# lrm2017/Fastest_Image_Pattern_Matching

Measured on AMD Instinct MI355X. Metric: template matches/sec + ms/search, 4024×3036 src ±180°; HBM GB/s vs roofline, higher is better.
Workload: dtype u8

## Files before the change

### fastest_image_pattern_matching_amd/csrc/fpm_engine.hip

```cpp
#include <hip/hip_runtime.h>

#include <algorithm>
#include <array>
#include <cfloat>
#include <chrono>
#include <cmath>
#include <cstdio>
#include <cstdlib>
#include <cstring>
#include <new>
#include <random>
#include <string>
#include <vector>

#include "../../include/fpm.h"
#include "fpm_host.h"
#include "fpm_kernels.h"
#include "fpm_model.h"

using namespace fpm;

namespace {

inline int round_up(int v, int a) { return (v + a - 1) / a * a; }
// ... 64 lines not shown
    std::vector<size_t> node_off;
    F2 center;
    std::vector<size_t> canvas_off, map_off, blk_off;
    std::vector<int> canvas_pitch, map_w, map_h, nblk;
    std::vector<int32_t> order;
    size_t canvas_bytes = 0, map_floats = 0, blk_count = 0;
    int max_canvas = 0, max_map = 0, max_nblk = 0, max_cells = 0, max_nitems = 0;
    NmsMaxima nmax;
    int off_skey = 0, nzero = 0;
    bool top_mma = false;
    TopMmaArgs tma{};
    int tcand_cap = 0;
    DevBuf d_tmu, d_tcandv;
    DevBuf d_ncand;
    DevBuf d_canvas, d_map, d_bmax, d_bloc, d_jobs, d_nodes, d_top, d_topn, d_peaks, d_counts, d_state,
        d_live, d_livecnt, d_rec, d_rowsum, d_wsum, d_wsq, d_tab, d_roi, d_tdesc, d_state2, d_rec2;
    int tabw = 0, tabh = 0, roi_pitch = 0, tdesc_stride = 1;
    size_t roi_stride = 0;
    int slot_cap = 0;
    size_t off_warp = 0, off_ncc = 0, off_nms = 0, off_order = 0;
    PinBuf h_out;
    size_t h_counts = 0, h_peaks = 0, h_live = 0, h_live0 = 0, h_state = 0, h_rec = 0, h_total = 0;
    char* h_dev = nullptr;
    void release() {
        for (DevBuf* b : {&d_tmu, &d_tcandv, &d_ncand, &d_canvas, &d_map, &d_bmax, &d_bloc, &d_jobs, &d_nodes, &d_top, &d_topn, &d_peaks,
                          &d_counts, &d_state, &d_live, &d_livecnt, &d_rec, &d_rowsum, &d_wsum, &d_wsq, &d_tab, &d_roi, &d_tdesc, &d_state2, &d_rec2})
            b->release();
        h_out.release();
        valid = false;
    }
};

struct RawPose {
    float x, y;
    double angle;
};

struct KProf {
    std::vector<std::pair<hipEvent_t, hipEvent_t>> ev;
    size_t used = 0;
    double ms = 0;
// ... 11 lines not shown
    bool learned = false;
    int border = 0;
    std::vector<TmplLevel> tmpl;
    DevBuf d_tmpl, d_tmpl8, d_tsum;
    uint64_t tmpl_gen = 0;
    int S = 0, sw = 0, sh = 0, src_L = -1;
    int shard = 0, shards = 1;
    std::vector<SrcLevel> src;
    DevBuf d_src;
    PinBuf h_imgtab;
    DevBuf d_imgtab;
    hipEvent_t in_ev = nullptr;
    Plan plan;
    uint64_t plan_gen = ~0ull;
    DevBuf d_op_a, d_op_b, d_op_job;
    DevBuf d_rf_tab, d_rf_tdesc, d_rf_roi, d_rf_rowsum, d_rf_wsum, d_rf_wsq;
    DevBuf d_ov;
    PinBuf h_ov_in, h_ov_out;
    std::vector<int64_t> stats;
    int64_t alg_bytes[3] = {0, 0, 0};
    bool prof = false;
    KProf kp[kProfSlots];
    hipGraphExec_t graph = nullptr;
    uint64_t graph_plan = ~0ull;
    const void* graph_src = nullptr;
    uint64_t plan_builds = 0;
    hipEvent_t t_ev[2] = {nullptr, nullptr};
    double last_device_ms = 0, last_host_ms = 0, last_call_ms = 0;
    std::chrono::steady_clock::time_point t_call0;
    bool pending = false;
    bool staged = false;
// ... 131 lines not shown
    n.cn = std::cos(-r); n.sn = std::sin(-r);
    return n;
}

SrcLevel level_layout(int w, int h) {
    SrcLevel s{};
    s.w = w; s.h = h;
    s.pitch = round_up(w + 4, 64);
    s.img_bytes = round_up((size_t)s.pitch * (h + 1), (size_t)256);
    return s;
}
size_t level_slab_slack(int pitch0) { return 16 * (size_t)pitch0 + 256; }

struct RoiScratchDims {
    int tabw = 1, tabh = 1, roi_pitch = 1, tdesc_stride = 1;
    size_t roi_stride = 0, max_rows = 1, max_chunks = 1;
    size_t per_roi() const {
        return sizeof(int32_t) * 2 * (tabw + tabh) + sizeof(int4) * tdesc_stride + roi_stride + max_rows * 49 * 4 +
               max_chunks * 49 * 12;
    }
};
RoiScratchDims roi_scratch_dims(const TmplLevel* lv, int nlv) {
    RoiScratchDims d;
    int max_w = 1;
    for (int l = 0; l < nlv; ++l) {
        d.tdesc_stride = std::max(d.tdesc_stride, roi_tiles_for(lv[l].w, lv[l].h));
        const int rc = roi_pick_rc(lv[l].w, lv[l].h);
        d.max_rows = std::max(d.max_rows, (size_t)lv[l].h);
        d.max_chunks = std::max(d.max_chunks, (size_t)(lv[l].h + rc - 1) / rc);
        max_w = std::max(max_w, lv[l].w);
        d.roi_stride = std::max(d.roi_stride, roi_tiles_bytes(lv[l].w, lv[l].h));
    }
    d.roi_pitch = roi_pitch_for(max_w);
    d.tabw = d.roi_pitch;
    d.tabh = roi_tab_rows((int)d.max_rows);
    return d;
}
hipError_t roi_scratch_ensure(const RoiScratchDims& d, size_t slots, DevBuf& tab, DevBuf& tdesc, DevBuf& roi,
                              DevBuf& rowsum, DevBuf& wsum, DevBuf& wsq) {
    hipError_t e = tab.ensure(slots * 2 * (d.tabw + d.tabh) * sizeof(int32_t));
    if (e == hipSuccess) e = tdesc.ensure(slots * d.tdesc_stride * sizeof(int4));
    if (e == hipSuccess) e = roi.ensure(slots * d.roi_stride);
    if (e == hipSuccess) e = rowsum.ensure(slots * round_up(d.max_rows * 49, (size_t)4) * 4);
    if (e == hipSuccess) e = wsum.ensure(slots * d.max_chunks * 49 * 4);
    if (e == hipSuccess) e = wsq.ensure(slots * d.max_chunks * 49 * 8);
    return e;
}

bool same_search_params(const fpm_params& a, const fpm_params& b) {
    return a.max_pos == b.max_pos && a.min_reduce_area == b.min_reduce_area && a.max_overlap == b.max_overlap &&
           a.score == b.score && a.tolerance_angle == b.tolerance_angle && a.use_simd == b.use_simd &&
           a.tolerance_range == b.tolerance_range && a.semantics == b.semantics &&
           a.top_angle_step == b.top_angle_step && std::equal(a.tolerance, a.tolerance + 4, b.tolerance) &&
           (a.stop_layer != 0) == (b.stop_layer != 0);
}

constexpr double kMaxTopAngles = 100000;
static bool angle_list_ok(const fpm_params& prm, double step, bool mfc) {
    if (!std::isfinite(step) || step <= 0) return false;
    auto span = [&](double lo, double hi) { return (hi - lo) / step + 2; };
// ... 246 lines not shown
        P.tabw = rd.tabw;
        P.tabh = rd.tabh;
        P.roi_stride = rd.roi_stride;
        const size_t per_roi = rd.per_roi();
        size_t free_b = 0, total_b = 0;
        if (hipMemGetInfo(&free_b, &total_b) != hipSuccess) free_b = (size_t)16 << 30;
        size_t budget = std::min((size_t)48 << 30, std::max(std::min((size_t)4 << 30, free_b / 2), free_b / 6));
        if (const char* e = getenv("FPM_SCRATCH_MB")) {
            const long mb = atol(e);
            if (mb > 0) budget = std::min(budget, (size_t)mb << 20);
        }
        const size_t want = (size_t)P.C * P.n3;
        P.slot_cap = (int)std::max<size_t>((size_t)P.n3, std::min(want, budget / per_roi) / P.n3 * P.n3);
        for (;;) {
            const hipError_t e = roi_scratch_ensure(rd, (size_t)P.slot_cap, P.d_tab, P.d_tdesc, P.d_roi, P.d_rowsum,
                                                    P.d_wsum, P.d_wsq);
            if (e == hipSuccess) break;
            (void)hipGetLastError();
            if (e != hipErrorOutOfMemory || P.slot_cap <= P.n3) HIP_TRY(e);
            P.d_tab.release(); P.d_tdesc.release(); P.d_roi.release();
            P.d_rowsum.release(); P.d_wsum.release(); P.d_wsq.release();
            P.slot_cap = std::max(P.n3, P.slot_cap / 2 / P.n3 * P.n3);
        }
    }
    std::vector<WarpJob> wj(J);
    std::vector<NccJob> nj(J);
    std::vector<NmsJob> mj(J);
    const uint8_t* dsrc = ctx->d_src.as<uint8_t>();
    for (int s = 0; s < S; ++s)
        for (int a = 0; a < P.nang; ++a) {
            const int k = s * P.nang + a;
            uint8_t* canvas = P.d_canvas.as<uint8_t>() + P.canvas_bytes * s + P.canvas_off[a];
            float* map = P.d_map.as<float>() + P.map_floats * s + P.map_off[a];
            WarpJob& w = wj[k];
            w.src = dsrc + top.off + top.img_bytes * s;
            w.sw = top.w; w.sh = top.h; w.sp = top.pitch;
// ... 294 lines not shown
    const char* stab_env = getenv("FPM_STEP_TABLES");
    const bool step_tables = (stab_env ? atoi(stab_env) != 0 : true) && (size_t)P.C * P.n3 <= (size_t)P.slot_cap;
    bool tables_done = false;
    for (int l = L - 1; l >= stop; --l) {
        const int d = L - 1 - l;
        const SrcLevel& lv = ctx->src[l];
        const TmplLevel& tl = ctx->tmpl[l];
        const bool in_run = l >= run_end;
        RoiArgs ra{};
        ra.level = dsrc + lv.off; ra.level_stride = lv.img_bytes;
        ra.W = lv.w; ra.H = lv.h; ra.P = lv.pitch;
        ra.tmpl = ctx->d_tmpl.as<uint8_t>() + tl.off; ra.tw = tl.w; ra.th = tl.h; ra.tp = tl.pitch;
        ra.tmpl8 = ctx->d_tmpl8.as<int8_t>() + tl.off8; ra.tp8 = tl.p8; ra.nk = (tl.w + 63) / 64;
        ra.tsum = ctx->d_tsum.as<int32_t>() + tl.tsum_off;
        ra.n3 = P.n3;
        ra.rc = roi_pick_rc(tl.w, tl.h);
        ra.nchunk = (tl.h + ra.rc - 1) / ra.rc;
        ra.fold = ctx->prm.use_simd ? 1 : 0;
        ra.equal1 = tl.equal1 ? 1 : 0;
        ra.per_source = P.nang * P.cap;
        ra.mean = tl.mean; ra.norm = tl.norm; ra.inv_area = tl.inv_area;
        ra.live = live[cur_list];
        ra.live_count = livecnt + list_cnt;
        ra.state = P.d_state.as<CandState>();
        ra.nodes = P.d_nodes.as<AngleNode>() + P.node_off[d];
        ra.tab = P.d_tab.as<int32_t>(); ra.tabw = roi_pitch_for(tl.w); ra.tabh = roi_tab_rows(tl.h);
        ra.tdesc = P.d_tdesc.as<int4>(); ra.tdesc_stride = P.tdesc_stride;
        ra.roi = P.d_roi.as<uint8_t>(); ra.roi_pitch = roi_pitch_for(tl.w); ra.roi_stride = P.roi_stride;
        ra.rowsum = P.d_rowsum.as<uint32_t>();
        ra.wsum = P.d_wsum.as<uint32_t>();
        ra.wsq = P.d_wsq.as<uint64_t>();
        ra.rec = P.d_rec.as<RoiRecord>();
        ra.step = l > stop ? 1 : 0;
        ra.mark_reached0 = l - 1 == stop ? 1 : 0;
        ra.live_out = live[cur_list ^ 1];
        ra.live_out_count = livecnt + d + 1;
        ra.thr = P.layer_score[l];
        if (in_run) {
            ra.rec = rec_buf[run_k & 1];
            if (run_k > 0) {
                ra.state = state_buf[(run_k + 1) & 1];
                ra.state_out = state_buf[run_k & 1];
                ra.prev_rec = rec_buf[(run_k + 1) & 1];
                ra.prev_nodes = P.d_nodes.as<AngleNode>() + P.node_off[d - 1];
                ra.prev_thr = P.layer_score[l + 1];
                ra.prev_W = ctx->src[l + 1].w;
// ... 1517 lines not shown
    }
    *out = ctx;
    return FPM_OK;
}

int fpm_destroy(fpm_ctx* ctx) {
    if (!ctx) return FPM_E_INVALID_ARG;
    (void)hipSetDevice(ctx->device);
    (void)hipStreamSynchronize(ctx->stream);
    if (ctx->graph) (void)hipGraphExecDestroy(ctx->graph);
    for (hipEvent_t e : ctx->t_ev)
        if (e) (void)hipEventDestroy(e);
    ctx->plan.release();
    ctx->d_tmpl.release(); ctx->d_tmpl8.release(); ctx->d_tsum.release(); ctx->d_src.release();
    ctx->d_op_a.release(); ctx->d_op_b.release(); ctx->d_op_job.release();
    for (DevBuf* b : {&ctx->d_rf_tab, &ctx->d_rf_tdesc, &ctx->d_rf_roi, &ctx->d_rf_rowsum, &ctx->d_rf_wsum, &ctx->d_rf_wsq})
        b->release();
    ctx->d_ov.release(); ctx->h_ov_in.release(); ctx->h_ov_out.release();
    ctx->d_imgtab.release(); ctx->h_imgtab.release();
    if (ctx->in_ev) (void)hipEventDestroy(ctx->in_ev);
    ctx->d_patchtab.release(); ctx->h_patchtab.release(); ctx->d_patch.release();
    ctx->d_cmpacc.release(); ctx->h_cmpacc.release();
    ctx->d_tacc.release(); ctx->h_tacc.release();
    ctx->d_model.release(); ctx->d_band.release(); ctx->d_insacc.release(); ctx->h_insacc.release();
    ctx->d_alnacc.release(); ctx->h_alnacc.release();
    for (hipEvent_t e : {ctx->tab_ev, ctx->out_ev})
        if (e) (void)hipEventDestroy(e);
    for (auto& k : ctx->kp)
        for (auto& e : k.ev) { (void)hipEventDestroy(e.first); (void)hipEventDestroy(e.second); }
    (void)hipStreamDestroy(ctx->stream);
    delete ctx;
// ... 1017 lines not shown
    hl[C] = C;
    const size_t o_state = 0, o_live = round_up(sizeof(CandState) * C, (size_t)256),
                 o_nodes = o_live + round_up(sizeof(int32_t) * (C + 1), (size_t)256),
                 o_rec = o_nodes + round_up(sizeof(AngleNode) * total_rois, (size_t)256);
    HIP_TRY(ctx->d_op_b.ensure(o_rec + sizeof(RoiRecord) * (size_t)total_rois));
    HIP_TRY(hipMemcpyAsync(ctx->d_op_b.as<char>(o_state), hs.data(), sizeof(CandState) * C, hipMemcpyHostToDevice, st));
    HIP_TRY(hipMemcpyAsync(ctx->d_op_b.as<char>(o_live), hl.data(), sizeof(int32_t) * (C + 1), hipMemcpyHostToDevice, st));
    HIP_TRY(hipMemcpyAsync(ctx->d_op_b.as<char>(o_nodes), hn.data(), sizeof(AngleNode) * total_rois, hipMemcpyHostToDevice,
                           st));
    HIP_TRY(hipMemsetAsync(ctx->d_op_b.as<char>(o_rec), 0, sizeof(RoiRecord) * (size_t)total_rois, st));
    const int slot_cap = round_rois > 0 ? std::min(round_rois, total_rois) : total_rois;
    const bool small = roi_small_fits(tl.w, tl.h);
    const RoiScratchDims rd = roi_scratch_dims(&tl, 1);
    if (!small)
        HIP_TRY(roi_scratch_ensure(rd, (size_t)slot_cap, ctx->d_rf_tab, ctx->d_rf_tdesc, ctx->d_rf_roi, ctx->d_rf_rowsum,
                                   ctx->d_rf_wsum, ctx->d_rf_wsq));
    RoiArgs ra{};
    ra.level = ctx->d_op_a.as<uint8_t>(); ra.level_stride = lv.img_bytes;
    ra.W = lv.w; ra.H = lv.h; ra.P = lv.pitch;
    ra.tmpl = ctx->d_tmpl.as<uint8_t>() + tl.off; ra.tw = tl.w; ra.th = tl.h; ra.tp = tl.pitch;
    ra.tmpl8 = ctx->d_tmpl8.as<int8_t>() + tl.off8; ra.tp8 = tl.p8; ra.nk = (tl.w + 63) / 64;
    ra.tsum = ctx->d_tsum.as<int32_t>() + tl.tsum_off;
    ra.n3 = n3;
    ra.rc = roi_pick_rc(tl.w, tl.h);
    ra.nchunk = (tl.h + ra.rc - 1) / ra.rc;
    ra.fold = fold ? 1 : 0;
    ra.equal1 = tl.equal1 ? 1 : 0;
    ra.per_source = n;
    ra.mean = tl.mean; ra.norm = tl.norm; ra.inv_area = tl.inv_area;
    ra.live = ctx->d_op_b.as<int32_t>(o_live);
    ra.live_count = ra.live + C;
    ra.state = ctx->d_op_b.as<CandState>(o_state);
    ra.nodes = ctx->d_op_b.as<AngleNode>(o_nodes);
    ra.tab = ctx->d_rf_tab.as<int32_t>(); ra.tabw = roi_pitch_for(tl.w); ra.tabh = roi_tab_rows(tl.h);
    ra.tdesc = ctx->d_rf_tdesc.as<int4>(); ra.tdesc_stride = rd.tdesc_stride;
    ra.roi = ctx->d_rf_roi.as<uint8_t>(); ra.roi_pitch = roi_pitch_for(tl.w); ra.roi_stride = rd.roi_stride;
    ra.rowsum = ctx->d_rf_rowsum.as<uint32_t>();
    ra.wsum = ctx->d_rf_wsum.as<uint32_t>();
    ra.wsq = ctx->d_rf_wsq.as<uint64_t>();
    ra.rec = ctx->d_op_b.as<RoiRecord>(o_rec);
    ra.step = 0;
    const bool want_px = roi_pixels && !small && !tl.equal1;
    const int RW = tl.w + 6, RH = tl.h + 6, txn = (RW + 31) / 32;
    std::vector<uint8_t> tiles;
    for (int base = 0; base < total_rois; base += slot_cap) {
        ra.slot_base = base;
        ra.slot_cap = std::min(slot_cap, total_rois - base);
        if (small) {
            ProfScope ps(ctx, FPM_K_ROI_SMALL, 0);
            launch_roi_small(ra, st);
            continue;
        }
        {
            ProfScope ps(ctx, FPM_K_ROI_TABLES, 0);
// ... 426 lines not shown
```

### fastest_image_pattern_matching_amd/csrc/fpm_kernels.h

```cpp
#pragma once
#include <hip/hip_runtime.h>
#include <stdint.h>

#include "fpm_geom.h"

namespace fpm {

struct WarpJob {
    const uint8_t* src;
    uint8_t* dst;
    int32_t sw, sh, sp;
    int32_t dw, dh, dp;
    int32_t border;
    int32_t pad;
    double M[6];
};

struct NccJob {
    const uint8_t* img;
    const uint8_t* tmpl;
    float* out;
    int32_t iw, ih, ip;
    int32_t tw, th, tp;
    int32_t ow, oh;
// ... 62 lines not shown
    F2 center;
    int32_t refine;
};

struct RoiArgs {
    const uint8_t* level;
    size_t level_stride;
    int32_t W, H, P;
    const uint8_t* tmpl;
    int32_t tw, th, tp;
    const int8_t* tmpl8;
    int32_t tp8;
    int32_t nk;
    const int32_t* tsum;
    int32_t n3;
    int32_t rc;
    int32_t nchunk;
    int32_t fold;
    int32_t equal1;
    int32_t per_source;
    int32_t slot_base;
    int32_t slot_cap;
    double mean, norm, inv_area;
    const int32_t* live;
    const int32_t* live_count;
    CandState* state;
    const AngleNode* nodes;
    int32_t* tab;
    int32_t tabw, tabh;
    int4* tdesc;
    int32_t tdesc_stride;
    uint8_t* roi;
    int32_t roi_pitch;
    size_t roi_stride;
    int32_t nparts;
    uint32_t* rowsum;
    uint32_t* wsum;
    uint64_t* wsq;
    RoiRecord* rec;
    int32_t step;
    int32_t mark_reached0;
    int32_t* live_out;
    int32_t* live_out_count;
    double thr;
    const RoiRecord* prev_rec;
    const AngleNode* prev_nodes;
    double prev_thr;
    int32_t prev_W, prev_H;
    CandState* state_out;
    int32_t* nt_tab;
    const AngleNode* nt_nodes;
    int32_t nt_tabw, nt_tabh, nt_tw, nt_th, nt_W, nt_H;
    uint64_t* stamps;
// ... 199 lines not shown
                       NmsLaunchInfo* info = nullptr);
void launch_roi_tables(const RoiArgs& a, hipStream_t st);
void launch_roi_warp(const RoiArgs& a, hipStream_t st);
void launch_roi_corr(const RoiArgs& a, hipStream_t st);
void launch_roi_eval(const RoiArgs& a, hipStream_t st);
bool roi_small_fits(int tw, int th);
size_t roi_small_lds(int tw, int th);
void launch_roi_small(const RoiArgs& a, hipStream_t st);
void launch_cand_step(const RoiArgs& a, int max_items, hipStream_t st);
void launch_pack(const PackArgs& a, hipStream_t st);

struct OvRect { F2 c[4]; float w, h; };
constexpr int kOverlapMaxCand = 512;
void launch_overlap_pairs(const OvRect* r, const float4* box, int n, double max_overlap, int32_t* lists, int list_cap,
                          int32_t* offcnt, int32_t* meta, hipStream_t st);
int roi_pick_rc(int tw, int th);
int roi_pitch_for(int tw);
int roi_tab_rows(int th);
size_t roi_tiles_bytes(int tw, int th);
int roi_tiles_for(int tw, int th);
size_t roi_corr_lds(int roi_pitch, int tw, int rc);
constexpr int kMmaRows = 16;

}
```

### fastest_image_pattern_matching_amd/csrc/fpm_kernels.hip

```cpp
#include <float.h>
#include <stdio.h>
#include <stdlib.h>
#include <limits.h>

#include <map>
#include <mutex>
#include <type_traits>
#include <utility>

#include "../../include/fpm.h"
#include "fpm_kernels.h"
#include "fpm_model.h"
#include "fpm_rrect.h"

static void ensure_lds_attr(const void* fn, size_t bytes) {
    if (bytes <= 65536) return;
    int dev = 0;
    (void)hipGetDevice(&dev);
    static std::mutex mu;
    static std::map<std::pair<int, const void*>, size_t> done;
    std::lock_guard<std::mutex> lock(mu);
    size_t& cur = done[std::make_pair(dev, fn)];
    if (bytes <= cur) return;
    (void)hipFuncSetAttribute(fn, hipFuncAttributeMaxDynamicSharedMemorySize, (int)bytes);
// ... 2036 lines not shown
    const int mode = !fuse ? 0 : (ci->refine == 0 ? 1 : (ci->refine == 2 ? 3 : 2));
    if (fuse && zero && nzero > 0 && mode != 1) {
        std::fprintf(stderr, "fpm: launch_top_fused contract violated (counter zeroing with candidate-init mode %d)\n",
                     mode);
        std::abort();
    }
    const int grid = top_fused_grid(njobs_n);
    if (dump)
        hipLaunchKernelGGL(k_top_fused<true>, dim3(grid), dim3(kTopThreads), lds, st, wjobs, njobs, a, zero, nzero,
                           fuse ? *ci : cz, mode, order, njobs_n);
    else
        hipLaunchKernelGGL(k_top_fused<false>, dim3(grid), dim3(kTopThreads), lds, st, wjobs, njobs, a, zero, nzero,
                           fuse ? *ci : cz, mode, order, njobs_n);
}

constexpr int ROI_RC = kMmaRows;
constexpr int ROI_T = 32;
constexpr int ROI_FT = 4096;
constexpr int kFtPitch = 68;
constexpr int kTabShift = 6;
constexpr int kTabFrac = kAbBits + kTabShift;
constexpr int kTapShift = kTabFrac - kInterBits;
constexpr uint32_t kRoiFlip = 0x80808080u;

int roi_pick_rc(int , int th) { return th < ROI_RC ? th : ROI_RC; }

__host__ __device__ inline int roi_pitch_calc(int tw) {
    const int need_a = tw + 6 + 16, need_b = 64 * ((tw + 63) / 64) + 22;
    int q = ((need_a > need_b ? need_a : need_b) + 15) / 16;
    if ((q & 1) == 0) ++q;
    return q * 16;
}
int roi_pitch_for(int tw) { return roi_pitch_calc(tw); }
int roi_tab_rows(int th) { return (th + 6 + ROI_T - 1) / ROI_T * ROI_T; }
__host__ __device__ inline int roi_tab_row_pos(int y) { return (y & ~31) | ((y & 7) << 2) | ((y >> 3) & 3); }
size_t roi_tiles_bytes(int tw, int th) {
    return (size_t)((tw + 6 + ROI_T - 1) / ROI_T) * ((th + 6 + ROI_T - 1) / ROI_T) * ROI_T * ROI_T;
}

__host__ __device__ inline int tmpl_lds_pitch(int tp8) {
    int q = tp8 / 16;
    if ((q & 1) == 0) ++q;
    return q * 16;
}

size_t roi_corr_lds(int roi_pitch, int , int ) {
    constexpr int src_rows = 2 * kMmaRows + 6;
    return (size_t)src_rows * roi_pitch +
           sizeof(uint32_t) * (2 * src_rows + 2 * 7 * src_rows + 2 * kMmaRows + 2 * kMmaRows * 49) + 64;
}

__device__ __forceinline__ int roi_tap(const uint8_t* __restrict__ src, int sw, int sh, int sp, int X, int Y) {
    const int sx = sat_s16(X >> kInterBits), sy = sat_s16(Y >> kInterBits);
    const int fx = X & (kInterTab - 1), fy = Y & (kInterTab - 1);
    int v0, v1, v2, v3;
    if ((unsigned)sx < (unsigned)(sw - 1) && (unsigned)sy < (unsigned)(sh - 1)) {
        const uint8_t* p = src + (size_t)sy * sp + sx;
        v0 = p[0]; v1 = p[1]; v2 = p[sp]; v3 = p[sp + 1];
    } else if (sx >= sw || sx + 1 < 0 || sy >= sh || sy + 1 < 0) {
        return 0;
    } else {
// ... 1472 lines not shown
    p1 = __builtin_amdgcn_udot4(a1, 0x01010101u, p1, false);
    p1 = __builtin_amdgcn_udot4(b0, 0x01010101u, p1, false);
    p1 = __builtin_amdgcn_udot4(b1, 0x01010101u, p1, false);
    uint32_t m1 = __builtin_amdgcn_udot4(c0, 0x01010101u, 0u, false);
    m1 = __builtin_amdgcn_udot4(c1, 0x01010101u, m1, false);
    uint32_t p2 = __builtin_amdgcn_udot4(a0, a0, 0u, false);
    p2 = __builtin_amdgcn_udot4(a1, a1, p2, false);
    p2 = __builtin_amdgcn_udot4(b0, b0, p2, false);
    p2 = __builtin_amdgcn_udot4(b1, b1, p2, false);
    uint32_t m2 = __builtin_amdgcn_udot4(c0, c0, 0u, false);
    m2 = __builtin_amdgcn_udot4(c1, c1, m2, false);
    q1 = p1 - m1;
    q2 = p2 - m2;
}

#ifndef FPM_CORR_PRIO
#define FPM_CORR_PRIO 1
#endif
template <int MODE, int WPE, int NK = 0, bool PFR = true, int RS = 1, bool SE = false, bool DMA = false>
__global__ __launch_bounds__(256) __attribute__((amdgpu_waves_per_eu(WPE))) void k_roi_corr(RoiArgs a) {
    static_assert(!DMA || (NK > 0 && !PFR), "LDS-DMA staging replaces the register staging of the register-A form");
    static_assert(NK == 0 || MODE != 3, "the staging ablation belongs to the slot-major form");
    static_assert(RS == 1 || RS == 3 || RS == 4, "the row statistics' forms");
    static_assert(!SE || NK > 0, "the staged epilogue is flushed in the register-A form's staging phase");
    static_assert(RS < 3 || NK > 0, "the matrix-core row sums read the register-A form's staged rows, every byte defined");
    extern __shared__ __attribute__((aligned(16))) uint8_t smem[];
    const int tw = a.tw, th = a.th, RW = tw + 6;
    const int SBp = a.roi_pitch;
    uint8_t* const SB = smem;
    uint32_t* wi = (uint32_t*)(SB + (size_t)kBandSrc * SBp) + 2 * kBandSrc;
    uint32_t* wq = wi + kBandSrc * 7;
    uint32_t* lts = wq + kBandSrc * 7;
    uint32_t* rsb = lts + 2 * kMmaRows;
    const int tid = threadIdx.x, lane = tid & 63, wv = tid >> 6;
    const int nband = (th + kBandRows - 1) / kBandRows;
    const int rois = roi_count(a), items = rois * nband;
    const int q4 = SBp >> 4;
    const int nwr = (RW + 3) >> 2;
    const int g = lane >> 4, n = lane & 15;
    const int mt = wv & 1, nt = mt + (wv >> 1);
    const int txn = (RW + ROI_T - 1) / ROI_T;
    const int npad = max(0, (min(ROI_T * txn, 64 * a.nk) - 4 * nwr) >> 2);
    const XcdSplit xs = xcd_split(items);
    int it_lo = xs.lo + xs.k, it_hi = xs.hi, it_step = xs.nk;
// ... 126 lines not shown
            uint32_t* rw = (uint32_t*)(SB + (size_t)sr * SBp);
            if (npad > 0) {
                if (g3 < npad) rw[nwr + g3] = kRoiFlip;
                if (g3 + 4 < npad) rw[nwr + g3 + 4] = kRoiFlip;
            }
            const int wr = tw >> 2;
            const uint32_t l0 = rw[0], l1 = rw[1], x0 = rw[wr], x1 = rw[wr + 1], x2 = rw[wr + 2];
            uint32_t s1, s2;
            tile_row_sums<RS == 4>((const uint8_t*)rw + 16 * g3, a.nk, n3, s1, s2);
            s2 = (uint32_t)__shfl((int)s2, n3 + 16 * (n3 >> 2), 64);
            const uint32_t e0 = __builtin_amdgcn_alignbyte(x1, x0, (uint32_t)tw) ^ 0x80808080u;
            const uint32_t e1 = __builtin_amdgcn_alignbyte(x2, x1, (uint32_t)tw) ^ 0x80808080u;
            const uint64_t lo = (uint64_t)(l0 ^ 0x80808080u) | ((uint64_t)(l1 ^ 0x80808080u) << 32);
            const uint64_t hi = (uint64_t)e0 | ((uint64_t)e1 << 32);
            const int nf = min(6, 64 * a.nk - tw);
#pragma unroll
            for (int h = 0; h < 2; ++h) {
                const int dx = g3 + 4 * h;
                if (dx < 7 && row < nsrc) {
                    uint32_t q1, q2;
                    window_edges(lo, hi, dx, nf, q1, q2);
                    wi[row * 7 + dx] = s1 - q1;
                    wq[row * 7 + dx] = s2 - q2;
                }
            }
        }
        if (RS == 1 && MODE != 7 && tid < 4 * nsrc) {
            const int r = tid >> 2, qq = tid & 3;
            const int per = (nwr + 3) >> 2, k0 = qq * per, k1 = min(nwr, k0 + per);
            const uint32_t* row = (const uint32_t*)(SB + (size_t)r * SBp);
            uint32_t s1 = 0, s2 = 0;
            int k = k0;
            for (; k + 8 <= k1; k += 8) {
                uint32_t x[8];
#pragma unroll
                for (int u = 0; u < 8; ++u) x[u] = row[k + u] ^ 0x80808080u;
#pragma unroll
                for (int u = 0; u < 8; ++u) {
                    s1 = __builtin_amdgcn_udot4(x[u], 0x01010101u, s1, false);
                    s2 = __builtin_amdgcn_udot4(x[u], x[u], s2, false);
                }
// ... 17 lines not shown
                const int dx = qq + 4 * h;
                if (dx < 7) {
                    const uint32_t ml0 = dx >= 4 ? 0xffffffffu : (1u << (8 * dx)) - 1u;
                    const uint32_t ml1 = dx <= 4 ? 0u : (1u << (8 * (dx - 4))) - 1u;
                    const uint32_t mr0 = dx >= 4 ? 0u : ~((1u << (8 * dx)) - 1u);
                    const uint32_t mr1 = dx <= 4 ? 0xffffu : dx == 5 ? 0xff00u : 0u;
                    const uint32_t a0 = l0 & ml0, a1 = l1 & ml1, b0 = e0 & mr0, b1 = e1 & mr1;
                    uint32_t q1 = __builtin_amdgcn_udot4(a0, 0x01010101u, 0u, false);
                    q1 = __builtin_amdgcn_udot4(a1, 0x01010101u, q1, false);
                    q1 = __builtin_amdgcn_udot4(b0, 0x01010101u, q1, false);
                    q1 = __builtin_amdgcn_udot4(b1, 0x01010101u, q1, false);
                    uint32_t q2 = __builtin_amdgcn_udot4(a0, a0, 0u, false);
                    q2 = __builtin_amdgcn_udot4(a1, a1, q2, false);
                    q2 = __builtin_amdgcn_udot4(b0, b0, q2, false);
                    q2 = __builtin_amdgcn_udot4(b1, b1, q2, false);
                    wi[r * 7 + dx] = s1 - q1;
                    wq[r * 7 + dx] = s2 - q2;
                }
            }
        }
        __syncthreads();
        auto partials = [&]() {
            if (MODE == 6 || tid >= 4 * 49) return;
            const int pr = tid >> 1, half = tid & 1;
            const int h = pr / 49, k = pr - h * 49;
            const int chunk = (T0 >> 4) + h;
            const int tlo = kMmaRows * h, thi = min(tlo + kMmaRows, rb);
            const bool ok = chunk < a.nchunk && tlo < thi;
            const int pdy = k / 7, ddx = k - pdy * 7;
            const int t0 = tlo + 8 * half, n8 = ok ? min(8, thi - t0) : 0;
            uint32_t s1 = 0, x[8], y[8];
#pragma unroll
            for (int u = 0; u < 8; ++u) {
                const int i = (t0 + u + pdy) * 7 + ddx;
                x[u] = u < n8 ? wi[i] : 0u;
                y[u] = u < n8 ? wq[i] : 0u;
            }
            uint64_t s2 = 0;
#pragma unroll
            for (int u = 0; u < 8; ++u) { s1 += x[u]; s2 += y[u]; }
            s1 += (uint32_t)__builtin_amdgcn_mov_dpp((int)s1, 0xB1, 0xF, 0xF, false);
            const uint32_t lo = (uint32_t)s2, hi = (uint32_t)(s2 >> 32);
            s2 += (uint64_t)(uint32_t)__builtin_amdgcn_mov_dpp((int)lo, 0xB1, 0xF, 0xF, false) |
                  ((uint64_t)(uint32_t)__builtin_amdgcn_mov_dpp((int)hi, 0xB1, 0xF, 0xF, false) << 32);
            if (ok && half == 0) {
                uint32_t kk = (uint32_t)k;
                asm volatile("" : "+v"(kk));
                const uint32_t wo = ((uint32_t)slot * (uint32_t)a.nchunk + (uint32_t)chunk) * 49u + kk;
                a.wsum[wo] = s1;
                a.wsq[wo] = s2;
            }
        };
        const bool active = kMmaRows * mt < rb && kMmaRows * nt < nsrc;
        if (FPM_CORR_PRIO == 1) __builtin_amdgcn_s_setprio(1);
        if (MODE != 2 && active) {
            int sr = kMmaRows * nt + n;
            if (sr >= nsrc) sr = 0;
            const uint8_t* bp = SB + (size_t)sr * SBp + 16 * g;
            fpm_v4i acc[7];
            if (FPM_CORR_PRIO == 2) __builtin_amdgcn_s_setprio(1);
            if (NK > 0)
                band_mfma_regs<NA>(Areg, bp, a.nk, acc);
            else
                band_mfma_ga(a.tmpl8 + (size_t)(T0 + kMmaRows * mt + n) * a.tp8 + 16 * g, bp, a.nk, acc);
            if (FPM_CORR_PRIO == 2) __builtin_amdgcn_s_setprio(0);
            uint32_t* rs_out = a.rowsum + (((size_t)th * 49 + 3) & ~(size_t)3) * slot + (size_t)T0 * 49;
// ... 14 lines not shown
                        if (x == 0x9e3779b9u && a.W < 0) rs_out[t] = x;
                        continue;
                    }
                    const uint32_t o = (uint32_t)(t * 49 + dy * 7);
                    if (SE) {
#pragma unroll
                        for (int d = 0; d < 7; ++d) rsb[o + d] = (uint32_t)acc[d][r] + 128u * (wi[s_ * 7 + d] + ts) - kFix;
                        continue;
                    }
#pragma unroll
                    for (int d = 0; d < 7; ++d) rs_out[o + d] = (uint32_t)acc[d][r] + 128u * (wi[s_ * 7 + d] + ts) - kFix;
                }
            }
        }
        if (FPM_CORR_PRIO == 1) __builtin_amdgcn_s_setprio(0);
        partials();
        if (SE) { pv_slot = slot; pv_T0 = T0; pv_rb = rb; }
    }
    if (SE && pv_slot >= 0) {
        __syncthreads();
        flush();
    }
}

__device__ __forceinline__ CandState cand_step_state(CandState s, int n3, const AngleNode* nodes, double thr, int W,
                                                     int H, int mark_reached0, const float* score, const int* mx,
                                                     const int* my, const AngleNode* next_nodes = nullptr,
                                                     int jj = 0, AngleNode* next_nd = nullptr, int nnext = 1) {
    int imax = 0;
    double big = -1;
    for (int k = 0; k < n3; ++k)
// ... 479 lines not shown
                         RoiRecord* keep) {
    constexpr int kEvalRows = ROWS, kEvalDma = EvalBlk<ROWS>::dma, kEvalBuf = EvalBlk<ROWS>::buf;
    const int th = a.th;
    if (a.equal1) {
        if (lane == 0) {
            RoiRecord r;
            r.score = 1.f; r.mx = 0; r.my = 0; r.on_border = 1;
            for (int k = 0; k < 9; ++k) r.vec[k] = 0.f;
            *out = r;
            *keep = r;
        }
        return;
    }
    const size_t total4 = ((size_t)th * 49 + 3) >> 2;
    const uint4* rs = (const uint4*)(a.rowsum + (size_t)slot * total4 * 4);
    uint64_t s1 = 0, s2 = 0;
    if (lane < 49) {
        const uint32_t* ws = a.wsum + (size_t)slot * a.nchunk * 49 + lane;
        const uint64_t* wq = a.wsq + (size_t)slot * a.nchunk * 49 + lane;
        int c = 0;
        for (; c + 8 <= a.nchunk; c += 8) {
            uint32_t x[8];
            uint64_t y[8];
#pragma unroll
            for (int u = 0; u < 8; ++u) { x[u] = ws[(size_t)(c + u) * 49]; y[u] = wq[(size_t)(c + u) * 49]; }
#pragma unroll
            for (int u = 0; u < 8; ++u) { s1 += x[u]; s2 += y[u]; }
        }
        for (; c < a.nchunk; ++c) { s1 += ws[(size_t)c * 49]; s2 += wq[(size_t)c * 49]; }
    }
    constexpr int BQ = kEvalRows * 49 / 4;
    const int nblk = (th + kEvalRows - 1) / kEvalRows;
    auto issue_block = [&](int b, uint8_t* buf) {
#pragma unroll
        for (int i = 0; i < kEvalDma; ++i) {
            size_t q = (size_t)b * BQ + 64 * i + lane;
            if (64 * i + lane >= BQ || q >= total4) q = 0;
            uint32_t keep;
            const uint32_t ldsa = (uint32_t)(uintptr_t)(fpm_lds_vp)(buf + 1024 * i);
            asm volatile("s_mov_b32 %0, m0\n\ts_mov_b32 m0, %2\n\ts_nop 0\n\tglobal_load_lds_dwordx4 %1, off\n\ts_mov_b32 m0, %0"
                         : "=&s"(keep) : "v"(rs + q), "s"(__builtin_amdgcn_readfirstlane(ldsa)) : "memory");
        }
    };
    float accF = 0.f;
    uint64_t accI = 0;
    issue_block(0, blk);
    for (int b = 0; b < nblk; ++b) {
        const uint32_t* cb = (const uint32_t*)(blk + (b & 1) * kEvalBuf);
        if (b + 1 < nblk) {
            issue_block(b + 1, blk + ((b + 1) & 1) * kEvalBuf);
            asm volatile("s_waitcnt vmcnt(%0)" :: "i"(kEvalDma) : "memory");
        } else {
            asm volatile("s_waitcnt vmcnt(0)" ::: "memory");
        }
        wave_sync();
        const int rows = min(kEvalRows, th - b * kEvalRows);
        if (lane < 49) {
            if (a.fold) {
                int t = 0;
                for (; t + 8 <= rows; t += 8) {
                    uint32_t x[8];
// ... 121 lines not shown
        }
        if ((NK == 8 || NK == 12) && lds * 4 <= kLdsPerCu) {
            const int grid = capped((int)std::min<long>(items, 4L * device_cus()), grid_cap_env(getenv("FPM_GRID_CORR"), 0));
            hipLaunchKernelGGL((k_roi_corr<0, 4, NK, false, kRS, true, true>), dim3(grid), dim3(256), lds, st, a);
            return;
        }
        const int grid = capped((int)std::min<long>(items, (long)kCorrWaves * device_cus()), grid_cap_env(getenv("FPM_GRID_CORR"), 0));
        hipLaunchKernelGGL((k_roi_corr<0, kCorrWaves, NK, false, kRS, true>), dim3(grid), dim3(256), lds, st, a);
    } else {
        const int grid = (int)std::min<long>(items, (long)kCorrRunWaves * device_cus());
        hipLaunchKernelGGL((k_roi_corr<0, kCorrRunWaves, NK, true, kRS>), dim3(grid), dim3(256), lds, st, a);
    }
}
void launch_roi_corr(const RoiArgs& a, hipStream_t st) {
    if (a.slot_cap <= 0 || a.equal1) return;
    const size_t lds = roi_corr_lds(a.roi_pitch, a.tw, a.rc);
    if ((a.roi_pitch >> 4) <= 64 && a.nk <= 16 && lds <= 65536) {
        const long items = (long)a.slot_cap * ((a.th + kBandRows - 1) / kBandRows);
        if (a.nk <= 4) launch_corr_regs<4>(a, items, lds, st);
        else if (a.nk <= 8) launch_corr_regs<8>(a, items, lds, st);
        else if (a.nk <= 12) launch_corr_regs<12>(a, items, lds, st);
        else launch_corr_regs<16>(a, items, lds, st);
        return;
    }
    ensure_lds_attr((const void*)k_roi_corr<0, kCorrWaves>, lds);
    const long items = (long)a.slot_cap * ((a.th + kBandRows - 1) / kBandRows);
    const int grid = (int)(items < 16384 ? items : 16384);
    hipLaunchKernelGGL((k_roi_corr<0, kCorrWaves>), dim3(grid), dim3(256), lds, st, a);
}

void launch_roi_eval(const RoiArgs& a, hipStream_t st) {
// ... 587 lines not shown
```

Measured before the change: 36350.

## Replace per-chunk 49-offset window partials with per-band 7-column totals plus edge rows

The correlation kernel used to write 49 partial window sums (and sums of squares) per 16-row chunk to global memory, which the eval kernel then accumulated across chunks. It now writes only 7 per-column totals per 32-row band, reduced with DPP and shuffles, plus a small set of top and bottom edge rows per slot. The eval kernel rebuilds the 49 window sums from band totals and edge-row differences through wave shuffles. This is meant to cut global scratch traffic and the partials pass, at the cost of more intricate reconstruction logic and a tight coupling between band geometry and edge storage.

```diff
diff --git a/fastest_image_pattern_matching_amd/csrc/fpm_engine.hip b/fastest_image_pattern_matching_amd/csrc/fpm_engine.hip
--- a/fastest_image_pattern_matching_amd/csrc/fpm_engine.hip
+++ b/fastest_image_pattern_matching_amd/csrc/fpm_engine.hip
@@ -102,7 +102,7 @@
     DevBuf d_tmu, d_tcandv;
     DevBuf d_ncand;
     DevBuf d_canvas, d_map, d_bmax, d_bloc, d_jobs, d_nodes, d_top, d_topn, d_peaks, d_counts, d_state,
-        d_live, d_livecnt, d_rec, d_rowsum, d_wsum, d_wsq, d_tab, d_roi, d_tdesc, d_state2, d_rec2;
+        d_live, d_livecnt, d_rec, d_rowsum, d_wtot, d_wtotq, d_wedge, d_tab, d_roi, d_tdesc, d_state2, d_rec2;
     int tabw = 0, tabh = 0, roi_pitch = 0, tdesc_stride = 1;
     size_t roi_stride = 0;
     int slot_cap = 0;
@@ -112,7 +112,7 @@
     char* h_dev = nullptr;
     void release() {
         for (DevBuf* b : {&d_tmu, &d_tcandv, &d_ncand, &d_canvas, &d_map, &d_bmax, &d_bloc, &d_jobs, &d_nodes, &d_top, &d_topn, &d_peaks,
-                          &d_counts, &d_state, &d_live, &d_livecnt, &d_rec, &d_rowsum, &d_wsum, &d_wsq, &d_tab, &d_roi, &d_tdesc, &d_state2, &d_rec2})
+                          &d_counts, &d_state, &d_live, &d_livecnt, &d_rec, &d_rowsum, &d_wtot, &d_wtotq, &d_wedge, &d_tab, &d_roi, &d_tdesc, &d_state2, &d_rec2})
             b->release();
         h_out.release();
         valid = false;
@@ -154,7 +154,7 @@
     Plan plan;
     uint64_t plan_gen = ~0ull;
     DevBuf d_op_a, d_op_b, d_op_job;
-    DevBuf d_rf_tab, d_rf_tdesc, d_rf_roi, d_rf_rowsum, d_rf_wsum, d_rf_wsq;
+    DevBuf d_rf_tab, d_rf_tdesc, d_rf_roi, d_rf_rowsum, d_rf_wtot, d_rf_wtotq, d_rf_wedge;
     DevBuf d_ov;
     PinBuf h_ov_in, h_ov_out;
     std::vector<int64_t> stats;
@@ -316,10 +316,10 @@
 
 struct RoiScratchDims {
     int tabw = 1, tabh = 1, roi_pitch = 1, tdesc_stride = 1;
-    size_t roi_stride = 0, max_rows = 1, max_chunks = 1;
+    size_t roi_stride = 0, max_rows = 1, max_bands = 1;
     size_t per_roi() const {
         return sizeof(int32_t) * 2 * (tabw + tabh) + sizeof(int4) * tdesc_stride + roi_stride + max_rows * 49 * 4 +
-               max_chunks * 49 * 12;
+               max_bands * 7 * 12 + kRoiEdgeWords * 4;
     }
 };
 RoiScratchDims roi_scratch_dims(const TmplLevel* lv, int nlv) {
@@ -327,9 +327,8 @@
     int max_w = 1;
     for (int l = 0; l < nlv; ++l) {
         d.tdesc_stride = std::max(d.tdesc_stride, roi_tiles_for(lv[l].w, lv[l].h));
-        const int rc = roi_pick_rc(lv[l].w, lv[l].h);
         d.max_rows = std::max(d.max_rows, (size_t)lv[l].h);
-        d.max_chunks = std::max(d.max_chunks, (size_t)(lv[l].h + rc - 1) / rc);
+        d.max_bands = std::max(d.max_bands, (size_t)roi_bands(lv[l].h));
         max_w = std::max(max_w, lv[l].w);
         d.roi_stride = std::max(d.roi_stride, roi_tiles_bytes(lv[l].w, lv[l].h));
     }
@@ -339,13 +338,14 @@
     return d;
 }
 hipError_t roi_scratch_ensure(const RoiScratchDims& d, size_t slots, DevBuf& tab, DevBuf& tdesc, DevBuf& roi,
-                              DevBuf& rowsum, DevBuf& wsum, DevBuf& wsq) {
+                              DevBuf& rowsum, DevBuf& wtot, DevBuf& wtotq, DevBuf& wedge) {
     hipError_t e = tab.ensure(slots * 2 * (d.tabw + d.tabh) * sizeof(int32_t));
     if (e == hipSuccess) e = tdesc.ensure(slots * d.tdesc_stride * sizeof(int4));
     if (e == hipSuccess) e = roi.ensure(slots * d.roi_stride);
     if (e == hipSuccess) e = rowsum.ensure(slots * round_up(d.max_rows * 49, (size_t)4) * 4);
-    if (e == hipSuccess) e = wsum.ensure(slots * d.max_chunks * 49 * 4);
-    if (e == hipSuccess) e = wsq.ensure(slots * d.max_chunks * 49 * 8);
+    if (e == hipSuccess) e = wtot.ensure(slots * d.max_bands * 7 * 4);
+    if (e == hipSuccess) e = wtotq.ensure(slots * d.max_bands * 7 * 8);
+    if (e == hipSuccess) e = wedge.ensure(slots * kRoiEdgeWords * 4);
     return e;
 }
 
@@ -622,12 +622,12 @@
         P.slot_cap = (int)std::max<size_t>((size_t)P.n3, std::min(want, budget / per_roi) / P.n3 * P.n3);
         for (;;) {
             const hipError_t e = roi_scratch_ensure(rd, (size_t)P.slot_cap, P.d_tab, P.d_tdesc, P.d_roi, P.d_rowsum,
-                                                    P.d_wsum, P.d_wsq);
+                                                    P.d_wtot, P.d_wtotq, P.d_wedge);
             if (e == hipSuccess) break;
             (void)hipGetLastError();
             if (e != hipErrorOutOfMemory || P.slot_cap <= P.n3) HIP_TRY(e);
             P.d_tab.release(); P.d_tdesc.release(); P.d_roi.release();
-            P.d_rowsum.release(); P.d_wsum.release(); P.d_wsq.release();
+            P.d_rowsum.release(); P.d_wtot.release(); P.d_wtotq.release(); P.d_wedge.release();
             P.slot_cap = std::max(P.n3, P.slot_cap / 2 / P.n3 * P.n3);
         }
     }
@@ -952,8 +952,6 @@
         ra.tmpl8 = ctx->d_tmpl8.as<int8_t>() + tl.off8; ra.tp8 = tl.p8; ra.nk = (tl.w + 63) / 64;
         ra.tsum = ctx->d_tsum.as<int32_t>() + tl.tsum_off;
         ra.n3 = P.n3;
-        ra.rc = roi_pick_rc(tl.w, tl.h);
-        ra.nchunk = (tl.h + ra.rc - 1) / ra.rc;
         ra.fold = ctx->prm.use_simd ? 1 : 0;
         ra.equal1 = tl.equal1 ? 1 : 0;
         ra.per_source = P.nang * P.cap;
@@ -966,8 +964,9 @@
         ra.tdesc = P.d_tdesc.as<int4>(); ra.tdesc_stride = P.tdesc_stride;
         ra.roi = P.d_roi.as<uint8_t>(); ra.roi_pitch = roi_pitch_for(tl.w); ra.roi_stride = P.roi_stride;
         ra.rowsum = P.d_rowsum.as<uint32_t>();
-        ra.wsum = P.d_wsum.as<uint32_t>();
-        ra.wsq = P.d_wsq.as<uint64_t>();
+        ra.wtot = P.d_wtot.as<uint32_t>();
+        ra.wtotq = P.d_wtotq.as<uint64_t>();
+        ra.wedge = P.d_wedge.as<uint32_t>();
         ra.rec = P.d_rec.as<RoiRecord>();
         ra.step = l > stop ? 1 : 0;
         ra.mark_reached0 = l - 1 == stop ? 1 : 0;
@@ -2515,7 +2514,7 @@
     ctx->plan.release();
     ctx->d_tmpl.release(); ctx->d_tmpl8.release(); ctx->d_tsum.release(); ctx->d_src.release();
     ctx->d_op_a.release(); ctx->d_op_b.release(); ctx->d_op_job.release();
-    for (DevBuf* b : {&ctx->d_rf_tab, &ctx->d_rf_tdesc, &ctx->d_rf_roi, &ctx->d_rf_rowsum, &ctx->d_rf_wsum, &ctx->d_rf_wsq})
+    for (DevBuf* b : {&ctx->d_rf_tab, &ctx->d_rf_tdesc, &ctx->d_rf_roi, &ctx->d_rf_rowsum, &ctx->d_rf_wtot, &ctx->d_rf_wtotq, &ctx->d_rf_wedge})
         b->release();
     ctx->d_ov.release(); ctx->h_ov_in.release(); ctx->h_ov_out.release();
     ctx->d_imgtab.release(); ctx->h_imgtab.release();
@@ -3563,7 +3562,7 @@
     const RoiScratchDims rd = roi_scratch_dims(&tl, 1);
     if (!small)
         HIP_TRY(roi_scratch_ensure(rd, (size_t)slot_cap, ctx->d_rf_tab, ctx->d_rf_tdesc, ctx->d_rf_roi, ctx->d_rf_rowsum,
-                                   ctx->d_rf_wsum, ctx->d_rf_wsq));
+                                   ctx->d_rf_wtot, ctx->d_rf_wtotq, ctx->d_rf_wedge));
     RoiArgs ra{};
     ra.level = ctx->d_op_a.as<uint8_t>(); ra.level_stride = lv.img_bytes;
     ra.W = lv.w; ra.H = lv.h; ra.P = lv.pitch;
@@ -3571,8 +3570,6 @@
     ra.tmpl8 = ctx->d_tmpl8.as<int8_t>() + tl.off8; ra.tp8 = tl.p8; ra.nk = (tl.w + 63) / 64;
     ra.tsum = ctx->d_tsum.as<int32_t>() + tl.tsum_off;
     ra.n3 = n3;
-    ra.rc = roi_pick_rc(tl.w, tl.h);
-    ra.nchunk = (tl.h + ra.rc - 1) / ra.rc;
     ra.fold = fold ? 1 : 0;
     ra.equal1 = tl.equal1 ? 1 : 0;
     ra.per_source = n;
@@ -3585,8 +3582,9 @@
     ra.tdesc = ctx->d_rf_tdesc.as<int4>(); ra.tdesc_stride = rd.tdesc_stride;
     ra.roi = ctx->d_rf_roi.as<uint8_t>(); ra.roi_pitch = roi_pitch_for(tl.w); ra.roi_stride = rd.roi_stride;
     ra.rowsum = ctx->d_rf_rowsum.as<uint32_t>();
-    ra.wsum = ctx->d_rf_wsum.as<uint32_t>();
-    ra.wsq = ctx->d_rf_wsq.as<uint64_t>();
+    ra.wtot = ctx->d_rf_wtot.as<uint32_t>();
+    ra.wtotq = ctx->d_rf_wtotq.as<uint64_t>();
+    ra.wedge = ctx->d_rf_wedge.as<uint32_t>();
     ra.rec = ctx->d_op_b.as<RoiRecord>(o_rec);
     ra.step = 0;
     const bool want_px = roi_pixels && !small && !tl.equal1;
diff --git a/fastest_image_pattern_matching_amd/csrc/fpm_kernels.h b/fastest_image_pattern_matching_amd/csrc/fpm_kernels.h
--- a/fastest_image_pattern_matching_amd/csrc/fpm_kernels.h
+++ b/fastest_image_pattern_matching_amd/csrc/fpm_kernels.h
@@ -100,8 +100,6 @@
     int32_t nk;
     const int32_t* tsum;
     int32_t n3;
-    int32_t rc;
-    int32_t nchunk;
     int32_t fold;
     int32_t equal1;
     int32_t per_source;
@@ -121,8 +119,9 @@
     size_t roi_stride;
     int32_t nparts;
     uint32_t* rowsum;
-    uint32_t* wsum;
-    uint64_t* wsq;
+    uint32_t* wtot;
+    uint64_t* wtotq;
+    uint32_t* wedge;
     RoiRecord* rec;
     int32_t step;
     int32_t mark_reached0;
@@ -352,12 +351,13 @@
 constexpr int kOverlapMaxCand = 512;
 void launch_overlap_pairs(const OvRect* r, const float4* box, int n, double max_overlap, int32_t* lists, int list_cap,
                           int32_t* offcnt, int32_t* meta, hipStream_t st);
-int roi_pick_rc(int tw, int th);
 int roi_pitch_for(int tw);
 int roi_tab_rows(int th);
 size_t roi_tiles_bytes(int tw, int th);
 int roi_tiles_for(int tw, int th);
-size_t roi_corr_lds(int roi_pitch, int tw, int rc);
+size_t roi_corr_lds(int roi_pitch);
+constexpr int kRoiEdgeWords = 2 * 12 * 7;
+int roi_bands(int th);
 constexpr int kMmaRows = 16;
 
 }
diff --git a/fastest_image_pattern_matching_amd/csrc/fpm_kernels.hip b/fastest_image_pattern_matching_amd/csrc/fpm_kernels.hip
--- a/fastest_image_pattern_matching_amd/csrc/fpm_kernels.hip
+++ b/fastest_image_pattern_matching_amd/csrc/fpm_kernels.hip
@@ -2074,7 +2074,6 @@
                            fuse ? *ci : cz, mode, order, njobs_n);
 }
 
-constexpr int ROI_RC = kMmaRows;
 constexpr int ROI_T = 32;
 constexpr int ROI_FT = 4096;
 constexpr int kFtPitch = 68;
@@ -2083,8 +2082,6 @@
 constexpr int kTapShift = kTabFrac - kInterBits;
 constexpr uint32_t kRoiFlip = 0x80808080u;
 
-int roi_pick_rc(int , int th) { return th < ROI_RC ? th : ROI_RC; }
-
 __host__ __device__ inline int roi_pitch_calc(int tw) {
     const int need_a = tw + 6 + 16, need_b = 64 * ((tw + 63) / 64) + 22;
     int q = ((need_a > need_b ? need_a : need_b) + 15) / 16;
@@ -2092,6 +2089,7 @@
     return q * 16;
 }
 int roi_pitch_for(int tw) { return roi_pitch_calc(tw); }
+int roi_bands(int th) { return (th + 2 * kMmaRows - 1) / (2 * kMmaRows); }
 int roi_tab_rows(int th) { return (th + 6 + ROI_T - 1) / ROI_T * ROI_T; }
 __host__ __device__ inline int roi_tab_row_pos(int y) { return (y & ~31) | ((y & 7) << 2) | ((y >> 3) & 3); }
 size_t roi_tiles_bytes(int tw, int th) {
@@ -2104,7 +2102,7 @@
     return q * 16;
 }
 
-size_t roi_corr_lds(int roi_pitch, int , int ) {
+size_t roi_corr_lds(int roi_pitch) {
     constexpr int src_rows = 2 * kMmaRows + 6;
     return (size_t)src_rows * roi_pitch +
            sizeof(uint32_t) * (2 * src_rows + 2 * 7 * src_rows + 2 * kMmaRows + 2 * kMmaRows * 49) + 64;
@@ -3607,6 +3605,18 @@
     q2 = p2 - m2;
 }
 
+__device__ __forceinline__ uint32_t row16_sum(uint32_t v) {
+    v += (uint32_t)__builtin_amdgcn_mov_dpp((int)v, 0xB1, 0xF, 0xF, false);
+    v += (uint32_t)__builtin_amdgcn_mov_dpp((int)v, 0x4E, 0xF, 0xF, false);
+    v += (uint32_t)__builtin_amdgcn_mov_dpp((int)v, 0x141, 0xF, 0xF, false);
+    v += (uint32_t)__builtin_amdgcn_mov_dpp((int)v, 0x140, 0xF, 0xF, false);
+    return v;
+}
+__device__ __forceinline__ uint64_t row16_sum_wide(uint32_t v) {
+    const uint32_t lo = row16_sum(v & 0xffffu), hi = row16_sum(v >> 16);
+    return (uint64_t)lo + ((uint64_t)hi << 16);
+}
+
 #ifndef FPM_CORR_PRIO
 #define FPM_CORR_PRIO 1
 #endif
@@ -3621,6 +3631,9 @@
     const int tw = a.tw, th = a.th, RW = tw + 6;
     const int SBp = a.roi_pitch;
     uint8_t* const SB = smem;
+    uint64_t* bt2 = (uint64_t*)(SB + (size_t)kBandSrc * SBp);
+    uint32_t* bt1 = (uint32_t*)(bt2 + 16);
+    static_assert(16 * 2 + 16 <= 2 * kBandSrc, "bt2 / bt1 fit the words between the rows and wi");
     uint32_t* wi = (uint32_t*)(SB + (size_t)kBandSrc * SBp) + 2 * kBandSrc;
     uint32_t* wq = wi + kBandSrc * 7;
     uint32_t* lts = wq + kBandSrc * 7;
@@ -3777,17 +3790,45 @@
             const uint64_t lo = (uint64_t)(l0 ^ 0x80808080u) | ((uint64_t)(l1 ^ 0x80808080u) << 32);
             const uint64_t hi = (uint64_t)e0 | ((uint64_t)e1 << 32);
             const int nf = min(6, 64 * a.nk - tw);
+            const uint32_t eo = (uint32_t)slot * (uint32_t)kRoiEdgeWords;
+            uint32_t t1[2] = {0u, 0u}, t2[2] = {0u, 0u};
 #pragma unroll
             for (int h = 0; h < 2; ++h) {
                 const int dx = g3 + 4 * h;
                 if (dx < 7 && row < nsrc) {
                     uint32_t q1, q2;
                     window_edges(lo, hi, dx, nf, q1, q2);
-                    wi[row * 7 + dx] = s1 - q1;
-                    wq[row * 7 + dx] = s2 - q2;
-                }
-            }
-        }
+                    const uint32_t v1 = s1 - q1, v2 = s2 - q2;
+                    wi[row * 7 + dx] = v1;
+                    wq[row * 7 + dx] = v2;
+                    if (MODE != 6) {
+                        if (row < rb) { t1[h] = v1; t2[h] = v2; }
+                        if (band == 0 && row < 6) {
+                            const uint32_t o = eo + (uint32_t)(row * 7 + dx);
+                            a.wedge[o] = v1;
+                            a.wedge[o + 84u] = v2;
+                        }
+                        if (band == nband - 1 && row >= rb) {
+                            const uint32_t o = eo + (uint32_t)((6 + row - rb) * 7 + dx);
+                            a.wedge[o] = v1;
+                            a.wedge[o + 84u] = v2;
+                        }
+                    }
+                }
+            }
+            if (MODE != 6 && nt < 2) {
+#pragma unroll
+                for (int h = 0; h < 2; ++h) {
+                    const uint32_t r1 = row16_sum(t1[h]);
+                    const uint64_t r2 = row16_sum_wide(t2[h]);
+                    if (n3 == 0 && g3 + 4 * h < 7) {
+                        bt1[8 * nt + g3 + 4 * h] = r1;
+                        bt2[8 * nt + g3 + 4 * h] = r2;
+                    }
+                }
+            }
+        }
+        uint32_t u1[2] = {0u, 0u}, u2[2] = {0u, 0u};
         if (RS == 1 && MODE != 7 && tid < 4 * nsrc) {
             const int r = tid >> 2, qq = tid & 3;
             const int per = (nwr + 3) >> 2, k0 = qq * per, k1 = min(nwr, k0 + per);
@@ -3835,42 +3876,53 @@
                     q2 = __builtin_amdgcn_udot4(a1, a1, q2, false);
                     q2 = __builtin_amdgcn_udot4(b0, b0, q2, false);
                     q2 = __builtin_amdgcn_udot4(b1, b1, q2, false);
-                    wi[r * 7 + dx] = s1 - q1;
-                    wq[r * 7 + dx] = s2 - q2;
+                    const uint32_t v1 = s1 - q1, v2 = s2 - q2;
+                    wi[r * 7 + dx] = v1;
+                    wq[r * 7 + dx] = v2;
+                    if (MODE != 6) {
+                        if (r < rb) { u1[h] = v1; u2[h] = v2; }
+                        const uint32_t eo = (uint32_t)slot * (uint32_t)kRoiEdgeWords;
+                        if (band == 0 && r < 6) {
+                            const uint32_t o = eo + (uint32_t)(r * 7 + dx);
+                            a.wedge[o] = v1;
+                            a.wedge[o + 84u] = v2;
+                        }
+                        if (band == nband - 1 && r >= rb) {
+                            const uint32_t o = eo + (uint32_t)((6 + r - rb) * 7 + dx);
+                            a.wedge[o] = v1;
+                            a.wedge[o + 84u] = v2;
+                        }
+                    }
+                }
+            }
+        }
+        if (RS == 1 && MODE != 7 && MODE != 6 && wv < 2) {
+#pragma unroll
+            for (int h = 0; h < 2; ++h) {
+                uint32_t r1 = u1[h], lo = u2[h] & 0xffffu, hi = u2[h] >> 16;
+#pragma unroll
+                for (int m = 4; m <= 32; m <<= 1) {
+                    r1 += (uint32_t)__shfl_xor((int)r1, m, 64);
+                    lo += (uint32_t)__shfl_xor((int)lo, m, 64);
+                    hi += (uint32_t)__shfl_xor((int)hi, m, 64);
+                }
+                if (lane < 4 && lane + 4 * h < 7) {
+                    bt1[8 * wv + lane + 4 * h] = r1;
+                    bt2[8 * wv + lane + 4 * h] = (uint64_t)lo + ((uint64_t)hi << 16);
                 }
             }
         }
         __syncthreads();
-        auto partials = [&]() {
-            if (MODE == 6 || tid >= 4 * 49) return;
-            const int pr = tid >> 1, half = tid & 1;
-            const int h = pr / 49, k = pr - h * 49;
-            const int chunk = (T0 >> 4) + h;
-            const int tlo = kMmaRows * h, thi = min(tlo + kMmaRows, rb);
-            const bool ok = chunk < a.nchunk && tlo < thi;
-            const int pdy = k / 7, ddx = k - pdy * 7;
-            const int t0 = tlo + 8 * half, n8 = ok ? min(8, thi - t0) : 0;
-            uint32_t s1 = 0, x[8], y[8];
-#pragma unroll
-            for (int u = 0; u < 8; ++u) {
-                const int i = (t0 + u + pdy) * 7 + ddx;
-                x[u] = u < n8 ? wi[i] : 0u;
-                y[u] = u < n8 ? wq[i] : 0u;
-            }
-            uint64_t s2 = 0;
-#pragma unroll
-            for (int u = 0; u < 8; ++u) { s1 += x[u]; s2 += y[u]; }
-            s1 += (uint32_t)__builtin_amdgcn_mov_dpp((int)s1, 0xB1, 0xF, 0xF, false);
-            const uint32_t lo = (uint32_t)s2, hi = (uint32_t)(s2 >> 32);
-            s2 += (uint64_t)(uint32_t)__builtin_amdgcn_mov_dpp((int)lo, 0xB1, 0xF, 0xF, false) |
-                  ((uint64_t)(uint32_t)__builtin_amdgcn_mov_dpp((int)hi, 0xB1, 0xF, 0xF, false) << 32);
-            if (ok && half == 0) {
-                uint32_t kk = (uint32_t)k;
-                asm volatile("" : "+v"(kk));
-                const uint32_t wo = ((uint32_t)slot * (uint32_t)a.nchunk + (uint32_t)chunk) * 49u + kk;
-                a.wsum[wo] = s1;
-                a.wsq[wo] = s2;
-            }
+        auto band_totals = [&]() {
+            if (MODE == 6 || MODE == 7 || tid < 128 || tid >= 128 + 7) return;
+            uint32_t dx = (uint32_t)(tid - 128);
+            asm volatile("" : "+v"(dx));
+            const bool two = rb > kMmaRows;
+            const uint32_t s1 = bt1[dx] + (two ? bt1[8 + dx] : 0u);
+            const uint64_t s2 = bt2[dx] + (two ? bt2[8 + dx] : 0ull);
+            const uint32_t wo = ((uint32_t)slot * (uint32_t)nband + (uint32_t)band) * 7u + dx;
+            a.wtot[wo] = s1;
+            a.wtotq[wo] = s2;
         };
         const bool active = kMmaRows * mt < rb && kMmaRows * nt < nsrc;
         if (FPM_CORR_PRIO == 1) __builtin_amdgcn_s_setprio(1);
@@ -3915,7 +3967,7 @@
             }
         }
         if (FPM_CORR_PRIO == 1) __builtin_amdgcn_s_setprio(0);
-        partials();
+        band_totals();
         if (SE) { pv_slot = slot; pv_T0 = T0; pv_rb = rb; }
     }
     if (SE && pv_slot >= 0) {
@@ -4425,21 +4477,22 @@
     }
     const size_t total4 = ((size_t)th * 49 + 3) >> 2;
     const uint4* rs = (const uint4*)(a.rowsum + (size_t)slot * total4 * 4);
-    uint64_t s1 = 0, s2 = 0;
-    if (lane < 49) {
-        const uint32_t* ws = a.wsum + (size_t)slot * a.nchunk * 49 + lane;
-        const uint64_t* wq = a.wsq + (size_t)slot * a.nchunk * 49 + lane;
-        int c = 0;
-        for (; c + 8 <= a.nchunk; c += 8) {
-            uint32_t x[8];
-            uint64_t y[8];
-#pragma unroll
-            for (int u = 0; u < 8; ++u) { x[u] = ws[(size_t)(c + u) * 49]; y[u] = wq[(size_t)(c + u) * 49]; }
-#pragma unroll
-            for (int u = 0; u < 8; ++u) { s1 += x[u]; s2 += y[u]; }
-        }
-        for (; c < a.nchunk; ++c) { s1 += ws[(size_t)c * 49]; s2 += wq[(size_t)c * 49]; }
-    }
+    const int nt7 = 7 * ((th + kBandRows - 1) / kBandRows);
+    const uint32_t* wt = a.wtot + (size_t)slot * nt7;
+    const uint64_t* wtq = a.wtotq + (size_t)slot * nt7;
+    uint32_t bx[4];
+    uint64_t by[4];
+#pragma unroll
+    for (int u = 0; u < 4; ++u) {
+        const int i = lane + 63 * u;
+        const bool ok = lane < 63 && i < nt7;
+        bx[u] = ok ? wt[i] : 0u;
+        by[u] = ok ? wtq[i] : 0ull;
+    }
+    const uint32_t* we = a.wedge + (size_t)slot * kRoiEdgeWords;
+    const bool el = lane < 42;
+    const uint32_t eh1 = el ? we[lane] : 0u, et1 = el ? we[42 + lane] : 0u;
+    const uint32_t eh2 = el ? we[84 + lane] : 0u, et2 = el ? we[126 + lane] : 0u;
     constexpr int BQ = kEvalRows * 49 / 4;
     const int nblk = (th + kEvalRows - 1) / kEvalRows;
     auto issue_block = [&](int b, uint8_t* buf) {
@@ -4456,6 +4509,22 @@
     float accF = 0.f;
     uint64_t accI = 0;
     issue_block(0, blk);
+    uint64_t p1 = (uint64_t)bx[0] + bx[1] + bx[2] + bx[3], p2 = by[0] + by[1] + by[2] + by[3];
+    for (int i = lane + 4 * 63; lane < 63 && i < nt7; i += 63) { p1 += wt[i]; p2 += wtq[i]; }
+    const int kdy = lane < 49 ? lane / 7 : 0, kdx = lane < 49 ? lane - 7 * kdy : 0;
+    const int d1 = (int)(et1 - eh1), d2 = (int)(et2 - eh2);
+    uint64_t s1 = 0, s2 = 0;
+#pragma unroll 3
+    for (int m = 0; m < 9; ++m) {
+        const int src = kdx + 7 * m;
+        s1 += (uint64_t)(uint32_t)__shfl((int)(uint32_t)p1, src, 64) | ((uint64_t)(uint32_t)__shfl((int)(p1 >> 32), src, 64) << 32);
+        s2 += (uint64_t)(uint32_t)__shfl((int)(uint32_t)p2, src, 64) | ((uint64_t)(uint32_t)__shfl((int)(p2 >> 32), src, 64) << 32);
+    }
+#pragma unroll 3
+    for (int r = 0; r < 6; ++r) {
+        const int v1 = __shfl(d1, kdx + 7 * r, 64), v2 = __shfl(d2, kdx + 7 * r, 64);
+        if (r < kdy) { s1 += (uint64_t)(int64_t)v1; s2 += (uint64_t)(int64_t)v2; }
+    }
     for (int b = 0; b < nblk; ++b) {
         const uint32_t* cb = (const uint32_t*)(blk + (b & 1) * kEvalBuf);
         if (b + 1 < nblk) {
@@ -4607,7 +4676,7 @@
 }
 void launch_roi_corr(const RoiArgs& a, hipStream_t st) {
     if (a.slot_cap <= 0 || a.equal1) return;
-    const size_t lds = roi_corr_lds(a.roi_pitch, a.tw, a.rc);
+    const size_t lds = roi_corr_lds(a.roi_pitch);
     if ((a.roi_pitch >> 4) <= 64 && a.nk <= 16 && lds <= 65536) {
         const long items = (long)a.slot_cap * ((a.th + kBandRows - 1) / kBandRows);
         if (a.nk <= 4) launch_corr_regs<4>(a, items, lds, st);
```

Result: faster. 36820 (median of 6 runs) (+1.3%).
